# Skeletus/SC-GameEngine

Hardware: AMD Instinct MI355X
Metric: entities/sec world-tick (xform+broadphase+cull), 1M-entity world (higher is better)
Workload: dtype f32

## Files before the change

### sc_gameengine_amd/csrc/sc_tick_kernels.hip

```cpp
#include "sc_tick_internal.h"
#include <hip/hip_ext.h>
#include "../../include/sc_tick.h"


namespace sctick {

#ifndef SC_XFORM_OCC
#define SC_XFORM_OCC
#endif
#ifndef SC_ROW_STORE_POLICY
#define SC_ROW_STORE_POLICY 2
#endif
#ifndef SC_WAVE_CHAINS
#define SC_WAVE_CHAINS 1
#endif
#ifndef SC_PAIR_OCC
#define SC_PAIR_OCC __attribute__((amdgpu_waves_per_eu(5, 5)))
#endif
#ifndef SC_PX_STORE_POLICY_TILE
#define SC_PX_STORE_POLICY_TILE 2
#endif
#ifndef SC_PX_STORE_POLICY_TAIL
#define SC_PX_STORE_POLICY_TAIL 0
#endif
#ifndef SC_DIAG_CLASSED_TAIL
#define SC_DIAG_CLASSED_TAIL 0
#endif

struct Aff { float r0[4], r1[4], r2[4]; };

__device__ __forceinline__ bool dirtyBit(const uint32_t* __restrict__ bits, uint32_t i)
{
  return (bits[i >> 5] >> (i & 31u)) & 1u;
}

__device__ __forceinline__ float ldF(const DeviceState& d, uint32_t stream, uint32_t i)
{
  return *reinterpret_cast<const float*>(d.fslab + (stream * d.capBytes + i * 4u));
}
__device__ __forceinline__ uint32_t ldU(const DeviceState& d, uint32_t stream, uint32_t i)
{
  return *reinterpret_cast<const uint32_t*>(d.fslab + (stream * d.capBytes + i * 4u));
}
__device__ __forceinline__ float4 ldRow(const DeviceState& d, uint32_t row, uint32_t i)
{
  return *reinterpret_cast<const float4*>(d.rslab + (row * d.capBytes16 + i * 16u));
}
typedef float V4f __attribute__((ext_vector_type(4)));
__device__ __forceinline__ void stRow(const DeviceState& d, uint32_t row, uint32_t i, const float4& v)
{
  *reinterpret_cast<float4*>(d.rslab + (row * d.capBytes16 + i * 16u)) = v;
}
__device__ __forceinline__ void stRowPolicy(const DeviceState& d, uint32_t row, uint32_t i, const float4& v)
{
#if SC_ROW_STORE_POLICY == 0
  stRow(d, row, i, v);
#else
  const V4f x = { v.x, v.y, v.z, v.w };
  const uint32_t off = row * d.capBytes16 + i * 16u;
#if SC_ROW_STORE_POLICY == 1
  __builtin_nontemporal_store(x, reinterpret_cast<V4f*>(d.rslab + off));
#elif SC_ROW_STORE_POLICY == 2
  asm volatile("global_store_dwordx4 %0, %1, %2 sc1" : : "v"(off), "v"(x), "s"(d.rslab) : "memory");
#elif SC_ROW_STORE_POLICY == 3
  asm volatile("global_store_dwordx4 %0, %1, %2 sc0 sc1" : : "v"(off), "v"(x), "s"(d.rslab) : "memory");
#else
#error "SC_ROW_STORE_POLICY: 0 plain, 1 nt, 2 sc1, 3 sc0 sc1"
#endif
#endif
}
template <int kPolicy>
__device__ __forceinline__ void stPxPolicy(const DeviceState& d, uint32_t i, float v)
{
  static_assert(kPolicy == 0 || kPolicy == 2, "px store policy: 0 plain, 2 sc1");
  if constexpr (kPolicy == 0) d.px[i] = v;
  else asm volatile("global_store_dword %0, %1, %2 sc1" : : "v"(i * 4u), "v"(v), "s"(d.px) : "memory");
}

__device__ __forceinline__ Aff loadLocal(const DeviceState& d, uint32_t j, uint32_t lkj)
{
  const uint32_t triv = lkj >> 29;
  float sx = 0.0f, cx = 1.0f, sy = 0.0f, cy = 1.0f, sz = 0.0f, cz = 1.0f;
  if (!(triv & 1u)) { sx = ldF(d, kRSX, j); cx = ldF(d, kRCX, j); }
  if (!(triv & 2u)) { sy = ldF(d, kRSY, j); cy = ldF(d, kRCY, j); }
  if (!(triv & 4u)) { sz = ldF(d, kRSZ, j); cz = ldF(d, kRCZ, j); }
  const float kx = ldF(d, kSX, j), ky = ldF(d, kSY, j), kz = ldF(d, kSZ, j);
  const float a00 = cz * cy, a10 = sz * cy, a20 = -sy;
  const float a01 = -sz,     a11 = cz;
  const float a02 = cz * sy, a12 = sz * sy, a22 = cy;
  const float nsx = -sx;
  const float r01 = a01 * cx + a02 * sx, r11 = a11 * cx + a12 * sx, r21 = a22 * sx;
  const float r02 = a01 * nsx + a02 * cx, r12 = a11 * nsx + a12 * cx, r22 = a22 * cx;
  Aff L;
  L.r0[0] = a00 * kx; L.r0[1] = r01 * ky; L.r0[2] = r02 * kz; L.r0[3] = ldF(d, kPX, j);
  L.r1[0] = a10 * kx; L.r1[1] = r11 * ky; L.r1[2] = r12 * kz; L.r1[3] = ldF(d, kPY, j);
  L.r2[0] = a20 * kx; L.r2[1] = r21 * ky; L.r2[2] = r22 * kz; L.r2[3] = ldF(d, kPZ, j);
  return L;
}
struct LocalRaw { float sx, cx, sy, cy, sz, cz, kx, ky, kz, px, py, pz; };
__device__ __forceinline__ LocalRaw requestLocal(const DeviceState& d, uint32_t j, uint32_t lkj)
{
  const uint32_t triv = lkj >> 29;
  LocalRaw r;
  r.sx = 0.0f; r.cx = 1.0f; r.sy = 0.0f; r.cy = 1.0f; r.sz = 0.0f; r.cz = 1.0f;
  if (!(triv & 1u)) { r.sx = ldF(d, kRSX, j); r.cx = ldF(d, kRCX, j); }
  if (!(triv & 2u)) { r.sy = ldF(d, kRSY, j); r.cy = ldF(d, kRCY, j); }
  if (!(triv & 4u)) { r.sz = ldF(d, kRSZ, j); r.cz = ldF(d, kRCZ, j); }
  r.kx = ldF(d, kSX, j); r.ky = ldF(d, kSY, j); r.kz = ldF(d, kSZ, j);
  r.px = ldF(d, kPX, j); r.py = ldF(d, kPY, j); r.pz = ldF(d, kPZ, j);
  return r;
}
__device__ __forceinline__ Aff buildLocal(const LocalRaw& q)
{
  const float a00 = q.cz * q.cy, a10 = q.sz * q.cy, a20 = -q.sy;
  const float a01 = -q.sz,       a11 = q.cz;
  const float a02 = q.cz * q.sy, a12 = q.sz * q.sy, a22 = q.cy;
  const float nsx = -q.sx;
  const float r01 = a01 * q.cx + a02 * q.sx, r11 = a11 * q.cx + a12 * q.sx, r21 = a22 * q.sx;
  const float r02 = a01 * nsx + a02 * q.cx, r12 = a11 * nsx + a12 * q.cx, r22 = a22 * q.cx;
  Aff L;
  L.r0[0] = a00 * q.kx; L.r0[1] = r01 * q.ky; L.r0[2] = r02 * q.kz; L.r0[3] = q.px;
  L.r1[0] = a10 * q.kx; L.r1[1] = r11 * q.ky; L.r1[2] = r12 * q.kz; L.r1[3] = q.py;
  L.r2[0] = a20 * q.kx; L.r2[1] = r21 * q.ky; L.r2[2] = r22 * q.kz; L.r2[3] = q.pz;
  return L;
}

__device__ __forceinline__ void mulRow(const float p[4], const Aff& L, float out[4])
{
  out[0] = (p[0] * L.r0[0] + p[1] * L.r1[0]) + p[2] * L.r2[0];
  out[1] = (p[0] * L.r0[1] + p[1] * L.r1[1]) + p[2] * L.r2[1];
  out[2] = (p[0] * L.r0[2] + p[1] * L.r1[2]) + p[2] * L.r2[2];
  out[3] = ((p[0] * L.r0[3] + p[1] * L.r1[3]) + p[2] * L.r2[3]) + p[3];
}
__device__ __forceinline__ Aff mulAff(const Aff& P, const Aff& L)
{
  Aff W;
  mulRow(P.r0, L, W.r0); mulRow(P.r1, L, W.r1); mulRow(P.r2, L, W.r2);
  return W;
}

__device__ __forceinline__ Aff loadRows(const DeviceState& d, uint32_t j)
{
  const float4 a = ldRow(d, 0, j), b = ldRow(d, 1, j), c = ldRow(d, 2, j);
  Aff M;
  M.r0[0] = a.x; M.r0[1] = a.y; M.r0[2] = a.z; M.r0[3] = a.w;
  M.r1[0] = b.x; M.r1[1] = b.y; M.r1[2] = b.z; M.r1[3] = b.w;
  M.r2[0] = c.x; M.r2[1] = c.y; M.r2[2] = c.z; M.r2[3] = c.w;
  return M;
}
__device__ __forceinline__ void storeRows(const DeviceState& d, uint32_t j, const Aff& M)
{
  stRow(d, 0, j, make_float4(M.r0[0], M.r0[1], M.r0[2], M.r0[3]));
  stRow(d, 1, j, make_float4(M.r1[0], M.r1[1], M.r1[2], M.r1[3]));
  stRow(d, 2, j, make_float4(M.r2[0], M.r2[1], M.r2[2], M.r2[3]));
}
__device__ __forceinline__ void storeRowsPolicy(const DeviceState& d, uint32_t j, const Aff& M)
{
  stRowPolicy(d, 0, j, make_float4(M.r0[0], M.r0[1], M.r0[2], M.r0[3]));
  stRowPolicy(d, 1, j, make_float4(M.r1[0], M.r1[1], M.r1[2], M.r1[3]));
  stRowPolicy(d, 2, j, make_float4(M.r2[0], M.r2[1], M.r2[2], M.r2[3]));
}

__device__ __forceinline__ float fromLane(int src4, float v) { return __int_as_float(__builtin_amdgcn_ds_bpermute(src4, __float_as_int(v))); }
__device__ __forceinline__ Aff affFromLane(int src4, const Aff& M)
{
  Aff P;
#pragma unroll
  for (int c = 0; c < 4; ++c) { P.r0[c] = fromLane(src4, M.r0[c]); P.r1[c] = fromLane(src4, M.r1[c]); P.r2[c] = fromLane(src4, M.r2[c]); }
  return P;
}

struct BoundsCE { float cx, cy, cz, ex, ey, ez; };
__device__ __forceinline__ BoundsCE loadBounds(const DeviceState& d, uint32_t j)
{
  const float x0 = ldF(d, kBMINX, j), y0 = ldF(d, kBMINY, j), z0 = ldF(d, kBMINZ, j);
  const float x1 = ldF(d, kBMAXX, j), y1 = ldF(d, kBMAXY, j), z1 = ldF(d, kBMAXZ, j);
  BoundsCE b;
  b.cx = (x0 + x1) * 0.5f; b.cy = (y0 + y1) * 0.5f; b.cz = (z0 + z1) * 0.5f;
  b.ex = (x1 - x0) * 0.5f; b.ey = (y1 - y0) * 0.5f; b.ez = (z1 - z0) * 0.5f;
  return b;
}
typedef const __attribute__((address_space(4))) float* ConstF;
typedef const __attribute__((address_space(4))) uint32_t* ConstU;
__device__ __forceinline__ BoundsCE paletteBounds(ConstF e)
{
  const float x0 = e[0], y0 = e[1], z0 = e[2], x1 = e[3], y1 = e[4], z1 = e[5];
  BoundsCE b;
  b.cx = (x0 + x1) * 0.5f; b.cy = (y0 + y1) * 0.5f; b.cz = (z0 + z1) * 0.5f;
  b.ex = (x1 - x0) * 0.5f; b.ey = (y1 - y0) * 0.5f; b.ez = (z1 - z0) * 0.5f;
  return b;
}

__device__ __forceinline__ bool sphereVisibleAt(const Aff& M, const BoundsCE& b, ConstF fr)
{
  const float c0 = M.r0[0] * b.cx + M.r0[1] * b.cy + M.r0[2] * b.cz + M.r0[3];
  const float c1 = M.r1[0] * b.cx + M.r1[1] * b.cy + M.r1[2] * b.cz + M.r1[3];
  const float c2 = M.r2[0] * b.cx + M.r2[1] * b.cy + M.r2[2] * b.cz + M.r2[3];
  const float nx = M.r0[0] * M.r0[0] + M.r1[0] * M.r1[0] + M.r2[0] * M.r2[0];
  const float ny = M.r0[1] * M.r0[1] + M.r1[1] * M.r1[1] + M.r2[1] * M.r2[1];
  const float nz = M.r0[2] * M.r0[2] + M.r1[2] * M.r1[2] + M.r2[2] * M.r2[2];
  const float nyz = (ny < nz) ? nz : ny;
  const float maxScale = sqrtf((nx < nyz) ? nyz : nx);
  const float radius = sqrtf(b.ex * b.ex + b.ey * b.ey + b.ez * b.ez) * maxScale;
  bool out = false;
#pragma unroll
  for (int k = 0; k < 6; ++k) {
    const float dist = fr[4 * k] * c0 + fr[4 * k + 1] * c1 + fr[4 * k + 2] * c2 + fr[4 * k + 3];
    out = out || (dist < -radius);
  }
  return !out;
}

__device__ __forceinline__ void worldAabb(const Aff& M, const BoundsCE& b, float mn[3], float mx[3])
{
  const float c0 = M.r0[0] * b.cx + M.r0[1] * b.cy + M.r0[2] * b.cz + M.r0[3];
  const float c1 = M.r1[0] * b.cx + M.r1[1] * b.cy + M.r1[2] * b.cz + M.r1[3];
  const float c2 = M.r2[0] * b.cx + M.r2[1] * b.cy + M.r2[2] * b.cz + M.r2[3];
  const float h0 = fabsf(M.r0[0]) * b.ex + fabsf(M.r0[1]) * b.ey + fabsf(M.r0[2]) * b.ez;
  const float h1 = fabsf(M.r1[0]) * b.ex + fabsf(M.r1[1]) * b.ey + fabsf(M.r1[2]) * b.ez;
  const float h2 = fabsf(M.r2[0]) * b.ex + fabsf(M.r2[1]) * b.ey + fabsf(M.r2[2]) * b.ez;
  mn[0] = c0 - h0; mn[1] = c1 - h1; mn[2] = c2 - h2;
  mx[0] = c0 + h0; mx[1] = c1 + h1; mx[2] = c2 + h2;
}

__device__ __forceinline__ void colliderAabb(const Aff& M, const float4& s, uint32_t type, float mn[3], float mx[3])
{
  float pad = 0.0f;
  if (type != kColliderBox) {
    const float nx = M.r0[0] * M.r0[0] + M.r1[0] * M.r1[0] + M.r2[0] * M.r2[0];
    const float ny = M.r0[1] * M.r0[1] + M.r1[1] * M.r1[1] + M.r2[1] * M.r2[1];
    const float nz = M.r0[2] * M.r0[2] + M.r1[2] * M.r1[2] + M.r2[2] * M.r2[2];
    const float nyz = (type == kColliderSphere && nz < ny) ? ny : nz;
    pad = s.w * sqrtf((nx < nyz) ? nyz : nx);
  }
  const float h0 = fabsf(M.r0[0]) * s.x + fabsf(M.r0[1]) * s.y + fabsf(M.r0[2]) * s.z + pad;
  const float h1 = fabsf(M.r1[0]) * s.x + fabsf(M.r1[1]) * s.y + fabsf(M.r1[2]) * s.z + pad;
  const float h2 = fabsf(M.r2[0]) * s.x + fabsf(M.r2[1]) * s.y + fabsf(M.r2[2]) * s.z + pad;
  mn[0] = M.r0[3] - h0; mn[1] = M.r1[3] - h1; mn[2] = M.r2[3] - h2;
  mx[0] = M.r0[3] + h0; mx[1] = M.r1[3] + h1; mx[2] = M.r2[3] + h2;
}
__device__ __forceinline__ bool hasProxy(uint32_t type, bool hasBounds) { return type == kColliderBounds ? hasBounds : type != kColliderNone; }
__device__ __forceinline__ bool proxyAabb(const DeviceState& d, uint32_t i, uint32_t lk, const Aff& M, float mn[3], float mx[3])
{
  const uint32_t type = d.colType ? d.colType[i] : kColliderBounds;
  if (!hasProxy(type, (lk & kHasBounds) != 0u)) return false;
  if (type == kColliderBounds) { const BoundsCE b = loadBounds(d, i); worldAabb(M, b, mn, mx); }
  else colliderAabb(M, d.colShape[i], type, mn, mx);
  return true;
}

struct BinPlan { bool collide, big; float x0, z0; uint32_t nx, nz; };

__device__ __forceinline__ BinPlan planBins(const TickParams& p, const float mn[3], const float mx[3])
{
  BinPlan b; b.collide = false; b.big = false; b.x0 = b.z0 = 0.0f; b.nx = b.nz = 0;
  if (!(mn[0] == mn[0] && mn[1] == mn[1] && mn[2] == mn[2] && mx[0] == mx[0] && mx[1] == mx[1] && mx[2] == mx[2])) return b;
  b.collide = true;
  const float x0 = floorf(mn[0] * p.invSector) - p.binOx, x1 = floorf(mx[0] * p.invSector) - p.binOx;
  const float z0 = floorf(mn[2] * p.invSector) - p.binOz, z1 = floorf(mx[2] * p.invSector) - p.binOz;
  const float nx = x1 - x0 + 1.0f, nz = z1 - z0 + 1.0f;
  const bool ok = x0 >= 0.0f && z0 >= 0.0f && x1 < (float)p.binSX && z1 < (float)p.binSZ &&
                  nx >= 1.0f && nx <= 2.0f && nz >= 1.0f && nz <= 2.0f;
  if (!ok) { b.big = true; return b; }
  b.x0 = x0; b.z0 = z0; b.nx = (uint32_t)nx; b.nz = (uint32_t)nz;
  return b;
}

__device__ __forceinline__ void appendBig(const DeviceState& d, const TickParams& p, const float4& rmin, const float4& rmax)
{
  const uint32_t slot = atomicAdd(&d.counters[kCtrPar + 8u * p.parity + kCtrBig], 1u);
  if (slot >= p.bigCap) return;
  d.bigList[2u * (size_t)slot] = rmin;
  d.bigList[2u * (size_t)slot + 1u] = rmax;
}

__device__ __forceinline__ void queueCrowded(const DeviceState& d, const TickParams& p, uint32_t sector)
{
  const uint32_t at = atomicAdd(&d.counters[kCtrPar + 8u * p.parity + kCtrCrowdTail], 1u);
  const uint32_t sectors = p.binSX * p.binSZ;
  if (at < sectors) d.crowdQueue[p.parity * sectors + at] = sector;
}

__device__ __forceinline__ void binInsertLane(const DeviceState& d, const TickParams& p, uint32_t sector, const float4& rmin, const float4& rm)
{
  const uint32_t slot = atomicAdd(&d.binCount[sector], 1u);
  atomicOr(&d.binLayers[sector], __float_as_uint(rmin.w));
  if (slot < kBinCap) {
    float4* r = d.bins + 2u * ((size_t)sector * kBinCap + slot);
    r[0] = rmin; r[1] = rm;
  } else {
    if (slot == kBinCap) queueCrowded(d, p, sector);
    const uint32_t ctr = kCtrPar + 8u * p.parity;
    const uint32_t at = atomicAdd(&d.counters[ctr + kCtrSpill], 1u);
    if (at < p.ovfCap) {
      d.spill[2u * (size_t)at] = rmin; d.spill[2u * (size_t)at + 1u] = rm; d.spillSector[at] = sector;
      atomicMin(&d.ovfLo[sector], at); atomicMax(&d.ovfHi[sector], at + 1u);
    } else atomicAdd(&d.counters[ctr + kCtrBorderLost], 1u);
  }
}

__device__ __forceinline__ void nullRecord(float4& lo, float4& hi, uint32_t id = 0x00FFFFFFu)
{
  lo = make_float4(INFINITY, INFINITY, INFINITY, __uint_as_float(0u));
  hi = make_float4(-INFINITY, -INFINITY, -INFINITY, __uint_as_float(id));
}

__host__ __device__ __forceinline__ uint32_t layersThatCanMeet(uint32_t H, uint32_t V)
{
  V |= H;
  const bool meet = ((V & 0xFFFFu) & (H >> 16)) != 0u && ((H & 0xFFFFu) & (V >> 16)) != 0u;
  return meet ? 0xFFFFFFFFu : 0u;
}
__device__ __forceinline__ bool binWrittenEveryTick(uint32_t homeLayers, uint32_t sector, uint32_t binSX, uint32_t binSZ)
{
  const uint32_t gx = sector % binSX, gz = sector / binSX;
  return ((homeLayers & 0xFFFFu) & (homeLayers >> 16)) != 0u || gx == 0u || gz == 0u || gx + 1u == binSX || gz + 1u == binSZ;
}

__device__ __forceinline__ void spillLane(const DeviceState& d, const TickParams& p, uint32_t sector, uint32_t slot, const float4& rmin, const float4& rm)
{
  if (slot == kBinCap) queueCrowded(d, p, sector);
  const uint32_t ctr = kCtrPar + 8u * p.parity;
  const uint32_t at = atomicAdd(&d.counters[ctr + kCtrSpill], 1u);
  if (at < p.ovfCap) {
    d.spill[2u * (size_t)at] = rmin; d.spill[2u * (size_t)at + 1u] = rm; d.spillSector[at] = sector;
    atomicMin(&d.ovfLo[sector], at); atomicMax(&d.ovfHi[sector], at + 1u);
  } else atomicAdd(&d.counters[ctr + kCtrBorderLost], 1u);
}

template <uint32_t kHome, bool kColl>
__device__ __forceinline__ void binEntityWave(const DeviceState& d, const TickParams& p, uint32_t i, bool collider,
                                              const Aff& M, const BoundsCE& b, bool storeM, bool lazyOn, uint32_t tile0, uint32_t tile1, uint32_t ctype)
{
  float mn[3] = {0, 0, 0}, mx[3] = {0, 0, 0};
  BinPlan plan; plan.collide = false; plan.big = false; plan.x0 = plan.z0 = 0.0f; plan.nx = plan.nz = 0;
  float4 rmin = make_float4(0, 0, 0, 0), rmax = make_float4(0, 0, 0, 0);
  constexpr uint32_t mode = kHome;
  uint32_t hA = kNoHome, hB = 0xFFFFFFFFu;
  if (mode == kHomeUse && i < p.n) { hA = d.homeA[i]; hB = d.homeB[i]; }
  if (collider) {
    if (kColl && ctype != kColliderBounds) colliderAabb(M, d.colShape[i], ctype, mn, mx);
    else worldAabb(M, b, mn, mx);
    plan = planBins(p, mn, mx);
    rmin = make_float4(mn[0], mn[1], mn[2], __uint_as_float((tile0 & kTileLayersShared) ? tile1 : ldU(d, kLAYERS, i)));
    rmax = make_float4(mx[0], mx[1], mx[2], __uint_as_float(i | p.rankBits));
  }
  const bool want = plan.collide && !plan.big;
  const uint32_t sector = (uint32_t)plan.z0 * p.binSX + (uint32_t)plan.x0;
  const uint32_t lane = threadIdx.x & 63u;
  const bool atHome = want && hA == sector;
  const bool r0 = atHome && (hB & 0xFFu) != kNoSlot;
  const bool a0 = want && !r0;
  uint32_t slot = hB & kSlotMask;
  const bool stay = p.cleanStay != 0u && !storeM;
  const bool skip0 = r0 && ((hB & kSlotAlways) ? stay : lazyOn);
  float4 rm = rmax;
  rm.w = __uint_as_float(i | p.rankBits | kPrimary);
  const uint32_t myLay = __float_as_uint(rmin.w);

  const unsigned long long act = ballot64(a0);
  uint32_t myHead = lane, runEnd = lane + 1u;
  if (act) {
    const uint32_t key = a0 ? sector : 0xFFFFFFFFu;
    const uint32_t prev = __shfl_up(key, 1, 64);
    const bool head = a0 && (lane == 0 || prev != key);
    const unsigned long long heads = ballot64(head);
    const unsigned long long upto = (lane == 63u) ? ~0ull : ((2ull << lane) - 1ull);
    myHead = (63u - (uint32_t)__clzll(heads & upto)) & 63u;
    const unsigned long long above = (myHead == 63u) ? 0ull : ~((2ull << myHead) - 1ull);
    const unsigned long long ends = (heads | ~act) & above;
    runEnd = ends ? (uint32_t)__ffsll((long long)ends) - 1u : 64u;
    uint32_t lay = a0 ? myLay : 0u;
    const uint32_t headLay = (uint32_t)__shfl((int)lay, (int)myHead, 64);
    if (ballot64(a0 && headLay != lay)) {
#pragma unroll
      for (uint32_t o = 1; o < 64u; o <<= 1) {
        const uint32_t other = (uint32_t)__shfl_down((int)lay, o, 64);
        if (a0 && lane + o < runEnd) lay |= other;
      }
    }
    uint32_t base = 0;
    if (head) { base = atomicAdd(&d.binCount[sector], runEnd - lane); atomicOr(&d.binLayers[sector], lay); }
    if (storeM) storeRows(d, i, M);
    base = __shfl(base, myHead, 64);
    if (a0) slot = base + (lane - myHead);
  } else if (storeM) storeRows(d, i, M);
  if (want && slot < kBinCap && !skip0) {
    float4* r = d.bins + 2u * ((size_t)sector * kBinCap + slot);
    r[0] = rmin; r[1] = rm;
  }
  uint32_t learned = (want && slot < kBinCap) ? slot : kNoSlot;
  const bool c1 = want && plan.nx > 1u, c2 = want && plan.nz > 1u, c3 = c1 && c2;
  if (mode == kHomeUse) {
    const uint32_t sec1 = sector + 1u, sec2 = sector + p.binSX, sec3 = sec2 + 1u;
    const uint32_t b1 = (hB >> 8) & 0xFFu, b2 = (hB >> 16) & 0xFFu, b3 = hB >> 24;
    uint32_t q1 = b1 & kSlotMask, q2 = b2 & kSlotMask, q3 = b3 & kSlotMask;
    const bool h1 = atHome && b1 != kNoSlot, h2 = atHome && b2 != kNoSlot, h3 = atHome && b3 != kNoSlot;
    const bool a1 = c1 && !h1, a2 = c2 && !h2, a3 = c3 && !h3;
    const bool w1 = c1 && !(h1 && ((b1 & kSlotAlways) ? stay : lazyOn)), w2 = c2 && !(h2 && ((b2 & kSlotAlways) ? stay : lazyOn)),
               w3 = c3 && !(h3 && ((b3 & kSlotAlways) ? stay : lazyOn));
    if (a1) q1 = atomicAdd(&d.binCount[sec1], 1u);
    if (a2) q2 = atomicAdd(&d.binCount[sec2], 1u);
    if (a3) q3 = atomicAdd(&d.binCount[sec3], 1u);
    if (w1 && q1 < kBinCap) { float4* r = d.bins + 2u * ((size_t)sec1 * kBinCap + q1); r[0] = rmin; r[1] = rmax; }
    if (w2 && q2 < kBinCap) { float4* r = d.bins + 2u * ((size_t)sec2 * kBinCap + q2); r[0] = rmin; r[1] = rmax; }
    if (w3 && q3 < kBinCap) { float4* r = d.bins + 2u * ((size_t)sec3 * kBinCap + q3); r[0] = rmin; r[1] = rmax; }
    if (a1) atomicOr(&d.binLayers[sec1], myLay);
    if (a2) atomicOr(&d.binLayers[sec2], myLay);
    if (a3) atomicOr(&d.binLayers[sec3], myLay);
    if (ballot64((a1 && q1 >= kBinCap) || (a2 && q2 >= kBinCap) || (a3 && q3 >= kBinCap))) {
      if (a1 && q1 >= kBinCap) spillLane(d, p, sec1, q1, rmin, rmax);
      if (a2 && q2 >= kBinCap) spillLane(d, p, sec2, q2, rmin, rmax);
      if (a3 && q3 >= kBinCap) spillLane(d, p, sec3, q3, rmin, rmax);
    }
    if (hA != kNoHome && !(atHome && c1 && c2)) {
      float4 lo, hi; nullRecord(lo, hi, i | p.rankBits);
#pragma unroll
      for (uint32_t k = 0; k < 4u; ++k) {
        const bool ck = k == 0u ? want : (k == 1u ? c1 : (k == 2u ? c2 : c3));
        const uint32_t gk = (hB >> (8u * k)) & 0xFFu;
        if (gk != kNoSlot && !(atHome && ck) && !(lazyOn && !(gk & kSlotAlways))) {
          float4* r = d.bins + 2u * ((size_t)(hA + (k & 1u) + (k >> 1) * p.binSX) * kBinCap + (gk & kSlotMask)); r[0] = lo; r[1] = hi;
        }
      }
    }
  } else {
    const uint32_t sec1 = sector + 1u, sec2 = sector + p.binSX, sec3 = sec2 + 1u;
    uint32_t q1 = 0, q2 = 0, q3 = 0;
    if (c1) q1 = atomicAdd(&d.binCount[sec1], 1u);
    if (c2) q2 = atomicAdd(&d.binCount[sec2], 1u);
    if (c3) q3 = atomicAdd(&d.binCount[sec3], 1u);
    if (c1 && q1 < kBinCap) { float4* r = d.bins + 2u * ((size_t)sec1 * kBinCap + q1); r[0] = rmin; r[1] = rmax; }
    if (c2 && q2 < kBinCap) { float4* r = d.bins + 2u * ((size_t)sec2 * kBinCap + q2); r[0] = rmin; r[1] = rmax; }
    if (c3 && q3 < kBinCap) { float4* r = d.bins + 2u * ((size_t)sec3 * kBinCap + q3); r[0] = rmin; r[1] = rmax; }
    if (c1) atomicOr(&d.binLayers[sec1], myLay);
    if (c2) atomicOr(&d.binLayers[sec2], myLay);
    if (c3) atomicOr(&d.binLayers[sec3], myLay);
    learned |= ((c1 && q1 < kBinCap ? q1 : kNoSlot) << 8) | ((c2 && q2 < kBinCap ? q2 : kNoSlot) << 16) | ((c3 && q3 < kBinCap ? q3 : kNoSlot) << 24);
    if (ballot64((c1 && q1 >= kBinCap) || (c2 && q2 >= kBinCap) || (c3 && q3 >= kBinCap))) {
      if (c1 && q1 >= kBinCap) spillLane(d, p, sec1, q1, rmin, rmax);
      if (c2 && q2 >= kBinCap) spillLane(d, p, sec2, q2, rmin, rmax);
      if (c3 && q3 >= kBinCap) spillLane(d, p, sec3, q3, rmin, rmax);
    }
    if (mode == kHomeLearn && i < p.n) { d.homeA[i] = want ? sector : kNoHome; d.homeB[i] = learned; }
  }
  const bool over = a0 && slot >= kBinCap;
  const unsigned long long mo = ballot64(over);
  if (mo) {
    const uint32_t ctr = kCtrPar + 8u * p.parity;
    const uint32_t first = (uint32_t)__ffsll((long long)mo) - 1u;
    uint32_t at = 0;
    if (lane == first) at = atomicAdd(&d.counters[ctr + kCtrSpill], (uint32_t)__popcll(mo));
    at = __shfl(at, (int)first, 64) + (uint32_t)__popcll(mo & ((1ull << lane) - 1ull));
    if (over && slot == kBinCap) queueCrowded(d, p, sector);
    if (over && at < p.ovfCap) {
      d.spill[2u * (size_t)at] = rmin; d.spill[2u * (size_t)at + 1u] = rm; d.spillSector[at] = sector;
      if (slot == kBinCap || lane == myHead) atomicMin(&d.ovfLo[sector], at);
      if (lane + 1u == runEnd) atomicMax(&d.ovfHi[sector], at + 1u);
    } else if (over) atomicAdd(&d.counters[ctr + kCtrBorderLost], 1u);
  }
  if (plan.collide && plan.big) appendBig(d, p, rmin, rmax);
}

__device__ __forceinline__ void binBoxSingle(const DeviceState& d, const TickParams& p, uint32_t i, const float mn[3], const float mx[3])
{
  const BinPlan plan = planBins(p, mn, mx);
  const float4 rmin = make_float4(mn[0], mn[1], mn[2], __uint_as_float(ldU(d, kLAYERS, i)));
  float4 rmax = make_float4(mx[0], mx[1], mx[2], __uint_as_float(i | p.rankBits));
  if (!plan.collide) return;
  if (plan.big) { appendBig(d, p, rmin, rmax); return; }
  const uint32_t sx = (uint32_t)plan.x0, sz = (uint32_t)plan.z0;
  for (uint32_t k = 0; k < 4; ++k) {
    const uint32_t dx = k & 1u, dz = k >> 1;
    if (!(dx < plan.nx && dz < plan.nz)) continue;
    float4 rm = rmax; if (k == 0) rm.w = __uint_as_float(i | p.rankBits | kPrimary);
    binInsertLane(d, p, (sz + dz) * p.binSX + (sx + dx), rmin, rm);
  }
}

__device__ __forceinline__ void binEntitySingle(const DeviceState& d, const TickParams& p, uint32_t i, const Aff& M, const BoundsCE& b)
{
  float mn[3], mx[3];
  worldAabb(M, b, mn, mx);
  binBoxSingle(d, p, i, mn, mx);
}

template <bool kCull, bool kAabb, uint32_t kChain, uint32_t kHome, bool kColl, bool kTail = false>
__device__ __forceinline__ void xformCullBody(const DeviceState& d, const TickParams& p);

__device__ __forceinline__ void spanTail(const DeviceState& d, const TickParams& p, uint32_t begin, uint32_t end, uint32_t tid)
{
  if (begin >= end) return;
  const bool produce = (p.flags & SC_TICK_PRODUCE_NEXT) != 0;
  const uint32_t wBegin = begin >> 5, wEnd = (end + 31u) >> 5;
  const uint32_t w = wBegin + tid;
  const uint32_t wAt = w < wEnd ? w : wEnd - 1u;
  const uint32_t dw = d.dirty[wAt], uw = d.unreach[wAt];
  uint32_t rw = 0u;
  if (produce) rw = d.rootMask[wAt];
  constexpr uint32_t kBatch = 3;
  uint32_t rm[kBatch]; float x[kBatch];
  if (produce) {
#pragma unroll
    for (uint32_t u = 0; u < kBatch; ++u) {
      const uint32_t i = begin + u * kTile + tid;
      const uint32_t at = i < end ? i : end - 1u;
      rm[u] = d.rootMask[at >> 5];
      x[u] = d.px[at];
    }
  }
  __syncthreads();
  if (produce) {
#pragma unroll
    for (uint32_t u = 0; u < kBatch; ++u) {
      const uint32_t i = begin + u * kTile + tid;
      if (i < end && ((rm[u] >> (i & 31u)) & 1u)) stPxPolicy<SC_PX_STORE_POLICY_TAIL>(d, i, x[u] + p.producerParam);
    }
    for (uint32_t base = begin + kBatch * kTile; base < end; base += kBatch * kTile) {
#pragma unroll
      for (uint32_t u = 0; u < kBatch; ++u) {
        const uint32_t i = base + u * kTile + tid;
        const uint32_t at = i < end ? i : end - 1u;
        rm[u] = d.rootMask[at >> 5];
        x[u] = d.px[at];
      }
#pragma unroll
      for (uint32_t u = 0; u < kBatch; ++u) {
        const uint32_t i = base + u * kTile + tid;
        if (i < end && ((rm[u] >> (i & 31u)) & 1u)) stPxPolicy<SC_PX_STORE_POLICY_TAIL>(d, i, x[u] + p.producerParam);
      }
    }
  }
  if (w < wEnd) d.dirty[w] = (dw & uw) | rw;
  for (uint32_t v = w + kTile; v < wEnd; v += kTile) d.dirty[v] = (d.dirty[v] & d.unreach[v]) | (produce ? d.rootMask[v] : 0u);
}

template <uint32_t kChain>
struct TileWalk {
  uint32_t lk;
  uint32_t a[kChain + 1];
  uint32_t rotFlags, cur;
  int top;
  uint32_t pendLink, pendDirty;
};
template <uint32_t kChain>
__device__ __forceinline__ void walkRequest(const DeviceState& d, TileWalk<kChain>& w, uint32_t i, uint32_t last)
{
  w.a[0] = i <= last ? i : last;
  w.pendLink = ldU(d, kLINK, w.a[0]);
  w.pendDirty = d.dirty[w.a[0] >> 5];
}
template <uint32_t kChain>
__device__ __forceinline__ void walkResolve(TileWalk<kChain>& w, uint32_t lev, uint32_t i, uint32_t last, bool doXform)
{
  asm volatile("" : : "v"(w.pendLink), "v"(w.pendDirty));
  if (lev == 0u) {
    w.lk = i <= last ? w.pendLink : ((kUnreachable << kDepthShift) | kNoParent);
    w.rotFlags = w.lk >> 29; w.cur = w.lk;
    const bool walk = doXform && linkDepth(w.lk) <= kChain;
    w.top = (walk && ((w.pendDirty >> (w.a[0] & 31u)) & 1u)) ? 0 : -1;
  } else {
    const uint32_t depth = linkDepth(w.lk);
    const bool on = doXform && depth <= kChain && lev <= depth;
    w.cur = on ? w.pendLink : w.cur;
    w.rotFlags |= on ? (w.pendLink >> 29) << (3u * lev) : 0u;
    w.top = (on && ((w.pendDirty >> (w.a[lev] & 31u)) & 1u)) ? (int)lev : w.top;
  }
}
template <uint32_t kChain>
__device__ __forceinline__ void walkIssue(const DeviceState& d, TileWalk<kChain>& w, uint32_t lev, bool doXform)
{
  const uint32_t depth = linkDepth(w.lk);
  const bool on = doXform && depth <= kChain && lev <= depth;
  w.a[lev] = on ? (w.cur & kParentMask) : w.a[0];
  w.pendLink = ldU(d, kLINK, w.a[lev]);
  w.pendDirty = d.dirty[w.a[lev] >> 5];
}

struct ClassPend { uint32_t tw0; uint2 ent, dm; };
__device__ __forceinline__ void classRequest(const DeviceState& d, ClassPend& np, uint32_t i, uint32_t last)
{
  const uint32_t a0 = i <= last ? i : last;
  const uint32_t t = __builtin_amdgcn_readfirstlane(a0 >> 6);
  np.tw0 = ((ConstU)d.boundsPalette)[kPaletteCap * 8u + 2u * t];
  np.dm = *reinterpret_cast<const uint2*>(d.dirty + 2u * (a0 >> 6));
}
__device__ __forceinline__ void classIssue(const DeviceState& d, ClassPend& np, uint32_t lane)
{
  const uint32_t pat = (np.tw0 >> kTopoShift) & kTopoMask;
  const uint32_t at = pat ? (pat <= kTopoCap ? pat - 1u : kTopoCap - 1u) : 0u;
  np.ent = topoTable(d.boundsPalette)[at * 64u + lane];
}
template <uint32_t kChain>
__device__ __forceinline__ void classResolve(const ClassPend& np, TileWalk<kChain>& w, uint32_t i, uint32_t last, uint32_t lane)
{
  asm volatile("" : : "v"(np.ent.x), "v"(np.dm.x), "v"(np.dm.y));
  const uint32_t pat = (np.tw0 >> kTopoShift) & kTopoMask;
  const uint32_t x = (i <= last && pat != 0u) ? np.ent.x : (kTopoInactive & 0xFF000000u);
  w.a[0] = i <= last ? i : last;
  w.lk = x; w.rotFlags = x >> 29; w.cur = x;
  const uint32_t depth = linkDepth(x);
  const bool walk = depth <= kChain;
  const unsigned long long dm = ((unsigned long long)np.dm.y << 32) | np.dm.x;
  int top = (walk && ((dm >> lane) & 1ull)) ? 0 : -1;
#pragma unroll
  for (uint32_t lev = 1; lev <= kChain; ++lev) {
    const uint32_t anc = (x >> (6u * (lev - 1u))) & 63u;
    top = (walk && lev <= depth && ((dm >> anc) & 1ull)) ? (int)lev : top;
  }
  w.top = top;
  if (kChain >= 1) w.a[kChain >= 1 ? 1 : 0] = (w.a[0] & ~63u) + (x & 63u);
}

template <bool kCull, uint32_t kChain, bool kTail, uint32_t kBatch = kChain + 1, bool kClassed = false>
__device__ __forceinline__ void xformCullPipelined(const DeviceState& d, const TickParams& p, const uint32_t bid = blockIdx.x)
{
  static_assert(kBatch >= 1 && kBatch <= kChain + 1, "levels requested together");
  static_assert(!kClassed || (SC_WAVE_CHAINS && kChain >= 1), "the classed form is the cooperative form");
  const uint32_t lane = threadIdx.x & 63u;
  const uint32_t wave = threadIdx.x >> 6;
  const uint32_t begin = bid * p.span;
  const uint32_t end = (begin + p.span < p.n) ? begin + p.span : p.n;
  const bool doXform = kClassed || (p.flags & SC_TICK_XFORM) != 0;
  const bool wantCand = (p.flags & SC_TICK_CULLED_LIST) != 0;
  const bool hasDeep = !kClassed && (p.flags & kFlagHasDeep) != 0;
  constexpr bool kEndInTile = kClassed && kTail;
  const bool produce = kEndInTile && !SC_DIAG_CLASSED_TAIL && (p.flags & SC_TICK_PRODUCE_NEXT) != 0;
  uint32_t tailWave = 0;
  if (kTail && !kCull && !kEndInTile) tailWave = __builtin_amdgcn_readfirstlane(wave);

  uint32_t visCount = 0, candCount = 0;
  TileWalk<kChain> w, nw;
  ClassPend np; uint32_t tw0 = 0u;

  auto tile = [&](uint32_t base, auto hasNext) {
    constexpr bool kNext = decltype(hasNext)::value;
    const uint32_t i = base + threadIdx.x;
    const uint32_t last = end - 1u;
    const bool active = i < p.n;
    const uint32_t lk = w.lk;
    const uint32_t depth = linkDepth(lk);
    const int top = w.top;
    const bool recompute = top >= 0;
    const bool fromRoot = (uint32_t)top == depth;

    uint32_t rows = i;
#pragma unroll
    for (uint32_t k = 0; k < kChain; ++k) if ((uint32_t)top == k) rows = w.a[k + 1];
    Aff M;
    auto walkAhead = [&]() {
      if constexpr (kClassed) { if (kNext) classRequest(d, np, i + kTile, last); }
      else if (kNext) { walkRequest(d, nw, i + kTile, last); walkResolve(nw, 0u, i + kTile, last, doXform); if (kChain >= 1) walkIssue(d, nw, 1u, doXform); }
    };
#if SC_WAVE_CHAINS
    bool coop = kClassed;
    if (!kClassed && kChain >= 1) coop = ballot64(top >= 1 && (w.a[kChain >= 1 ? 1 : 0] >> 6) != (i >> 6)) == 0ull;
    if (coop) {
      LocalRaw own;
      const bool nudge = produce && depth == 0u;
      if (recompute ? (top == 0 && !fromRoot) : (kCull && active)) M = loadRows(d, rows);
      if (recompute) own = requestLocal(d, w.a[0], w.rotFlags << 29);
      else if (kEndInTile && nudge) own.px = ldF(d, kPX, i);
      walkAhead();
      if (recompute) {
        const Aff L = buildLocal(own);
        if (top == 0 && !fromRoot) M = mulAff(M, L);
        else M = L;
      }
      if constexpr (kEndInTile && !SC_DIAG_CLASSED_TAIL) {
        if (nudge) stPxPolicy<SC_PX_STORE_POLICY_TILE>(d, i, own.px + p.producerParam);
        const unsigned long long nd = ballot64(nudge);
        if ((lane & 31u) == 0u && active) d.dirty[i >> 5] = (uint32_t)(nd >> lane);
      }
      const int src4 = (int)((top >= 1 ? (w.a[kChain >= 1 ? 1 : 0] & 63u) : lane) << 2);
#pragma unroll
      for (int pass = 1; pass <= (int)kChain; ++pass) {
        if (ballot64(top == pass) != 0ull) {
          const Aff P = affFromLane(src4, M);
          if (top == pass) M = mulAff(P, M);
        }
      }
    } else
#endif
    {
      if (recompute ? !fromRoot : (kCull && active)) M = loadRows(d, rows);
      LocalRaw raw[kChain + 1];
#pragma unroll
      for (int lev = (int)kChain; lev > (int)kChain - (int)kBatch; --lev)
        if (lev <= top) raw[lev] = requestLocal(d, w.a[lev], (w.rotFlags >> (3 * lev)) << 29);
      walkAhead();

      if (recompute) {
#pragma unroll
        for (int lev = (int)kChain; lev >= 0; --lev) {
          if (lev <= top) {
            if (lev <= (int)kChain - (int)kBatch) raw[lev] = requestLocal(d, w.a[lev], (w.rotFlags >> (3 * lev)) << 29);
            const Aff L = buildLocal(raw[lev]);
            if (lev == top && fromRoot) M = L;
            else M = mulAff(M, L);
          }
        }
      }
    }
    if constexpr (kClassed) { if (kNext) classIssue(d, np, lane); }
    else if (kNext && kChain >= 2) { walkResolve(nw, 1u, i + kTile, last, doXform); walkIssue(d, nw, 2u, doXform); }
    if (recompute) storeRowsPolicy(d, i, M);

    if (hasDeep) {
      const unsigned long long rm = ballot64(recompute);
      if (lane == 0 && (base + wave * 64u) < p.n) d.recomp[(base >> 6) + wave] = rm;
    }
    if (!kClassed && kNext && kChain >= 3) { walkResolve(nw, 2u, i + kTile, last, doXform); walkIssue(d, nw, 3u, doXform); }

    if (kCull) {
      const bool cand = active && (lk & kHasMesh);
      const bool hb = active && (lk & kHasBounds);
      const uint32_t t = __builtin_amdgcn_readfirstlane((base >> 6) + wave);
      ConstU tw = (ConstU)d.boundsPalette + (kPaletteCap * 8u + 2u * t);
      const uint32_t cls = (kClassed ? tw0 : tw[0]) & kClassMask;
      BoundsCE b = {0, 0, 0, 0, 0, 0};
      if (cls < kPaletteCap) b = paletteBounds((ConstF)d.boundsPalette + 8u * cls);
      else if (hb) b = loadBounds(d, i);

      bool visible = cand;
      if (cand && hb && !p.freeze && p.frustumValid) {
        const float* fr = d.frustum;
        asm volatile("" : "+s"(fr));
        visible = sphereVisibleAt(M, b, (ConstF)fr);
      }
      if (!kClassed && doXform && depth > kChain && depth != kUnreachable) visible = false;
      const unsigned long long vm = ballot64(visible);
      const unsigned long long cm = ballot64(cand);
      if (lane == 0 && (base + wave * 64u) < p.n) {
        d.vis[(base >> 6) + wave] = vm;
        if (wantCand) d.cand[(base >> 6) + wave] = cm;
      }
      visCount += (uint32_t)__popcll(vm);
      candCount += (uint32_t)__popcll(cm);
    }
    if constexpr (kClassed) { if (kNext) { classResolve(np, w, i + kTile, last, lane); tw0 = np.tw0; } }
    else if (kNext) { walkResolve(nw, kChain, i + kTile, last, doXform); w = nw; }
  };

  if (begin < end) {
    const uint32_t i0 = begin + threadIdx.x, last = end - 1u;
    if constexpr (kClassed) { classRequest(d, np, i0, last); classIssue(d, np, lane); classResolve(np, w, i0, last, lane); tw0 = np.tw0; }
    else {
      walkRequest(d, w, i0, last);
#pragma unroll
      for (uint32_t k = 1; k <= kChain; ++k) { walkResolve(w, k - 1u, i0, last, doXform); walkIssue(d, w, k, doXform); }
      walkResolve(w, kChain, i0, last, doXform);
    }
    uint32_t base = begin;
    for (; base + kTile < end; base += kTile) tile(base, std::true_type{});
    tile(base, std::false_type{});
  }

  if (kCull) {
    __shared__ uint32_t sVis[kTile / 64], sCand[kTile / 64];
    if (lane == 0) { sVis[wave] = visCount; sCand[wave] = candCount; }
    __syncthreads();
    if (threadIdx.x == 0) {
      d.blockVis[bid] = sVis[0] + sVis[1] + sVis[2] + sVis[3];
      d.blockCand[bid] = sCand[0] + sCand[1] + sCand[2] + sCand[3];
    }
  }
  if constexpr (kTail && !kEndInTile) spanTail(d, p, begin, end, kCull ? (wave << 6) + lane : (tailWave << 6) + __builtin_amdgcn_mbcnt_hi(~0u, __builtin_amdgcn_mbcnt_lo(~0u, 0u)));
}

#if SC_WAVE_CHAINS
constexpr uint32_t pipelinedBatch(bool, uint32_t) { return 1u; }
#else
constexpr uint32_t pipelinedBatch(bool cull, uint32_t chain) { return (cull && chain == 3u) ? 3u : chain + 1u; }
#endif

template <bool kCull, bool kAabb, uint32_t kChain, uint32_t kHome>
__global__ __launch_bounds__(kTile) SC_XFORM_OCC void k_xform_cull(const DeviceState d, const TickParams p)
{
  if constexpr (kAabb) xformCullBody<kCull, kAabb, kChain, kHome, false>(d, p);
  else xformCullPipelined<kCull, kChain, false, pipelinedBatch(kCull, kChain)>(d, p);
}
template <bool kCull, uint32_t kChain, uint32_t kHome>
__global__ __launch_bounds__(kTile) SC_XFORM_OCC void k_xform_cull_colliders(const DeviceState d, const TickParams p) { xformCullBody<kCull, true, kChain, kHome, true>(d, p); }
template <bool kCull, bool kAabb, uint32_t kChain, uint32_t kHome>
__global__ __launch_bounds__(kTile) SC_XFORM_OCC void k_xform_cull_tail(const DeviceState d, const TickParams p)
{
  if constexpr (kAabb) xformCullBody<kCull, kAabb, kChain, kHome, false, true>(d, p);
  else xformCullPipelined<kCull, kChain, true, pipelinedBatch(kCull, kChain)>(d, p);
}
template <bool kCull, uint32_t kChain>
__global__ __launch_bounds__(kTile) SC_XFORM_OCC void k_xform_cull_classed(const DeviceState d, const TickParams p) { xformCullPipelined<kCull, kChain, false, 1u, true>(d, p); }
template <bool kCull, uint32_t kChain>
__global__ __launch_bounds__(kTile) SC_XFORM_OCC void k_xform_cull_classed_tail(const DeviceState d, const TickParams p) { xformCullPipelined<kCull, kChain, true, 1u, true>(d, p); }
template <bool kCull, uint32_t kChain, uint32_t kHome>
__global__ __launch_bounds__(kTile) SC_XFORM_OCC void k_xform_cull_colliders_tail(const DeviceState d, const TickParams p) { xformCullBody<kCull, true, kChain, kHome, true, true>(d, p); }

template <bool kCull, bool kAabb, uint32_t kChain, uint32_t kHome, bool kColl, bool kTail>
__device__ __forceinline__ void xformCullBody(const DeviceState& d, const TickParams& p)
{
  const uint32_t lane = threadIdx.x & 63u;
  const uint32_t wave = threadIdx.x >> 6;
  const uint32_t begin = blockIdx.x * p.span;
  const uint32_t end = (begin + p.span < p.n) ? begin + p.span : p.n;
  const bool doXform = (p.flags & SC_TICK_XFORM) != 0;
  const bool wantCand = (p.flags & SC_TICK_CULLED_LIST) != 0;
  const bool hasDeep = (p.flags & kFlagHasDeep) != 0;
  uint32_t tailWave = 0;
  if (kTail && !kCull) tailWave = __builtin_amdgcn_readfirstlane(wave);

  uint32_t visCount = 0, candCount = 0;
  bool lazyOn = false;
  if (kAabb) {
    lazyOn = kHome == kHomeUse && (p.lazy == 2u || (p.lazy == 1u && d.lazyCtl[0] == 0u));
  }

  for (uint32_t base = begin; base < end; base += kTile) {
    const uint32_t i = base + threadIdx.x;
    const bool active = i < p.n;
    const uint32_t lk = active ? ldU(d, kLINK, i) : ((kUnreachable << kDepthShift) | kNoParent);
    const uint32_t ownDirtyWord = (doXform && active) ? d.dirty[i >> 5] : 0u;
    const uint32_t depth = linkDepth(lk);
    const bool chain = depth <= kChain;
    uint32_t a[kChain + 1];
    uint32_t rotFlags = lk >> 29;
    a[0] = i;
    int top = -1;
    if (doXform && chain) {
      if ((ownDirtyWord >> (i & 31u)) & 1u) top = 0;
      uint32_t cur = lk;
#pragma unroll
      for (uint32_t k = 1; k <= kChain; ++k) {
        a[k] = i;
        if (k <= depth) {
          a[k] = cur & kParentMask;
          cur = ldU(d, kLINK, a[k]);
          rotFlags |= (cur >> 29) << (3u * k);
          if (dirtyBit(d.dirty, a[k])) top = (int)k;
        }
      }
    } else {
#pragma unroll
      for (uint32_t k = 1; k <= kChain; ++k) a[k] = i;
    }
    const bool recompute = top >= 0;

    Aff M;
    if (recompute) {
      const bool fromRoot = (uint32_t)top == depth;
      uint32_t seed = i;
#pragma unroll
      for (uint32_t k = 0; k < kChain; ++k) if ((uint32_t)top == k) seed = a[k + 1];
      if (!fromRoot) M = loadRows(d, seed);
#pragma unroll
      for (int lev = (int)kChain; lev >= 0; --lev) {
        if (lev <= top) {
          const Aff L = loadLocal(d, a[lev], (rotFlags >> (3 * lev)) << 29);
          if (lev == top && fromRoot) M = L;
          else M = mulAff(M, L);
        }
      }
      if (!kAabb) storeRows(d, i, M);
    } else if ((kCull || kAabb) && active) {
      M = loadRows(d, i);
    }

    if (hasDeep) {
      const unsigned long long rm = ballot64(recompute);
      if (lane == 0 && (base + wave * 64u) < p.n) d.recomp[(base >> 6) + wave] = rm;
    }

    if (kCull || kAabb) {
      const bool cand = active && (lk & kHasMesh);
      const bool hb = active && (lk & kHasBounds);
      uint32_t ctype = kColliderNone;
      if (kColl && active) ctype = d.colType[i];
      const uint32_t t = __builtin_amdgcn_readfirstlane((base >> 6) + wave);
      ConstU tw = (ConstU)d.boundsPalette + (kPaletteCap * 8u + 2u * t);
      const uint32_t tile0 = tw[0], tile1 = kAabb ? tw[1] : 0u;
      const uint32_t cls = tile0 & kClassMask;
      BoundsCE b = {0, 0, 0, 0, 0, 0};
      if (cls < kPaletteCap) b = paletteBounds((ConstF)d.boundsPalette + 8u * cls);
      else if (hb) b = loadBounds(d, i);

      if (kCull) {
        bool visible = cand;
        if (cand && hb && !p.freeze && p.frustumValid) {
          const float* fr = d.frustum;
          asm volatile("" : "+s"(fr));
          visible = sphereVisibleAt(M, b, (ConstF)fr);
        }
        if (doXform && depth > kChain && depth != kUnreachable) visible = false;
        const unsigned long long vm = ballot64(visible);
        const unsigned long long cm = ballot64(cand);
        if (lane == 0 && (base + wave * 64u) < p.n) {
          d.vis[(base >> 6) + wave] = vm;
          if (wantCand) d.cand[(base >> 6) + wave] = cm;
        }
        visCount += (uint32_t)__popcll(vm);
        candCount += (uint32_t)__popcll(cm);
      }
      if (kAabb) {
        const bool collider = (kColl ? hasProxy(ctype, hb) : hb) && !(doXform && depth > kChain && depth != kUnreachable);
        binEntityWave<kHome, kColl>(d, p, i, collider, M, b, recompute, lazyOn, tile0, tile1, ctype);
      }
    }
  }

  if (kAabb && blockIdx.x == 0 && threadIdx.x == 0) d.lazyCtl[1u + p.parity] = lazyOn ? 0u : 1u;
  if (kCull) {
    __shared__ uint32_t sVis[kTile / 64], sCand[kTile / 64];
    if (lane == 0) { sVis[wave] = visCount; sCand[wave] = candCount; }
    __syncthreads();
    if (threadIdx.x == 0) {
      d.blockVis[blockIdx.x] = sVis[0] + sVis[1] + sVis[2] + sVis[3];
      d.blockCand[blockIdx.x] = sCand[0] + sCand[1] + sCand[2] + sCand[3];
    }
  }
  if (kTail) spanTail(d, p, begin, end, kCull ? (wave << 6) + lane : (tailWave << 6) + __builtin_amdgcn_mbcnt_hi(~0u, __builtin_amdgcn_mbcnt_lo(~0u, 0u)));
}

template <bool kColl>
__device__ __forceinline__ void deepLevelBody(const DeviceState& d, const TickParams& p, const uint32_t* __restrict__ list, uint32_t count)
{
  const uint32_t t = blockIdx.x * kTile + threadIdx.x;
  if (t >= count) return;
  const uint32_t i = list[t];
  const uint32_t lk = ldU(d, kLINK, i);
  const uint32_t par = lk & kParentMask;
  bool nodeDirty = false;
  Aff M;
  if (p.flags & SC_TICK_XFORM) {
    nodeDirty = dirtyBit(d.dirty, i) || ((d.recomp[par >> 6] >> (par & 63u)) & 1ull);
    if (nodeDirty) {
      const Aff P = loadRows(d, par);
      const Aff L = loadLocal(d, i, lk);
      M = mulAff(P, L);
      storeRows(d, i, M);
      atomicOr((unsigned long long*)&d.recomp[i >> 6], 1ull << (i & 63u));
    }
  }
  if (!nodeDirty) M = loadRows(d, i);
  const bool hb = (lk & kHasBounds) != 0;
  BoundsCE b = {0, 0, 0, 0, 0, 0};
  if (hb) b = loadBounds(d, i);
  if (p.flags & SC_TICK_CULL) {
    bool visible = (lk & kHasMesh) != 0;
    if (visible && hb && !p.freeze && p.frustumValid) visible = sphereVisibleAt(M, b, (ConstF)d.frustum);
    if (visible) {
      atomicOr((unsigned long long*)&d.vis[i >> 6], 1ull << (i & 63u));
      atomicAdd(&d.blockVis[i / p.span], 1u);
    }
  }
  if (p.flags & SC_TICK_BROADPHASE) {
    if (kColl) { float mn[3], mx[3]; if (proxyAabb(d, i, lk, M, mn, mx)) binBoxSingle(d, p, i, mn, mx); }
    else if (hb) binEntitySingle(d, p, i, M, b);
  }
}
__global__ __launch_bounds__(kTile) void k_deep_level(const DeviceState d, const TickParams p, const uint32_t* __restrict__ list, uint32_t count) { deepLevelBody<false>(d, p, list, count); }
__global__ __launch_bounds__(kTile) void k_deep_level_colliders(const DeviceState d, const TickParams p, const uint32_t* __restrict__ list, uint32_t count) { deepLevelBody<true>(d, p, list, count); }

__device__ __forceinline__ bool nudgePosition(const DeviceState& d, uint32_t i, uint32_t n, float dx)
{
  const bool in = i < n;
  const uint32_t lk = in ? d.link[i] : ((kUnreachable << kDepthShift) | 1u);
  const float x = in ? d.px[i] : 0.0f;
  const bool root = in && (lk & kParentMask) == kNoParent && linkDepth(lk) != kUnreachable;
  if (root) d.px[i] = x + dx;
  return root;
}
__device__ __forceinline__ void markDirtyWave(const DeviceState& d, uint32_t i, uint32_t n, bool moved)
{
  const uint32_t lane = threadIdx.x & 63u;
  const unsigned long long m = ballot64(moved);
  const uint32_t mine = lane < 32u ? (uint32_t)m : (uint32_t)(m >> 32);
  if (i < n && (lane & 31u) == 0u && mine) d.dirty[i >> 5] |= mine;
}
struct LaneStep { bool ok; uint32_t lane; float s; float pos[3]; float dir[3]; };
__device__ __forceinline__ LaneStep advanceAlongLane(const LaneGraphDev& g, uint32_t lane, float s, float distance)
{
  LaneStep r; r.ok = false; r.lane = lane; r.s = s;
  r.pos[0] = r.pos[1] = r.pos[2] = 0.0f; r.dir[0] = r.dir[1] = r.dir[2] = 0.0f;
  if (lane == kInvalidLane || lane >= g.segments) return r;
  float remaining = distance; uint32_t current = lane; float currentS = s;
  for (uint32_t guard = 0; guard < 8u; ++guard) {
    const float4 A = g.segA[current], B = g.segB[current]; const uint4 C = g.segC[current];
    if (!C.y) return r;
    const float len = A.w;
    if (len <= 1e-5f) return r;
    const float available = len - currentS;
    if (remaining <= available) {
      currentS += remaining;
      r.pos[0] = A.x + B.x * currentS; r.pos[1] = A.y + B.y * currentS; r.pos[2] = A.z + B.z * currentS;
      r.dir[0] = B.x; r.dir[1] = B.y; r.dir[2] = B.z;
      r.lane = current; r.s = currentS; r.ok = true;
      return r;
    }
    remaining -= available; currentS = 0.0f;
    uint32_t best = kInvalidLane; float bestDot = -1.0f;
    const uint32_t c0 = g.nodeConnOff[C.x], c1 = g.nodeConnOff[C.x + 1u];
    for (uint32_t k = c0; k < c1; ++k) {
      const uint32_t segId = g.nodeConn[k];
      if (segId >= g.segments) continue;
      if (!g.segC[segId].y) continue;
      const float4 D = g.segB[segId];
      const float dot = B.x * D.x + B.y * D.y + B.z * D.z;
      if (dot > bestDot) { bestDot = dot; best = segId; }
    }
    if (best == kInvalidLane) {
      const float4 E = g.nodePos[C.x];
      r.pos[0] = E.x; r.pos[1] = E.y; r.pos[2] = E.z; r.dir[0] = B.x; r.dir[1] = B.y; r.dir[2] = B.z;
      r.lane = current; r.s = len; r.ok = true;
      return r;
    }
    current = best;
  }
  return r;
}

__device__ __forceinline__ uint32_t queryNearestLaneWave(const LaneGraphDev& g, float x, float y, float z, float& sOut)
{
  const uint32_t lane = threadIdx.x & 63u;
  float bestD = INFINITY, bestS = 0.0f; uint32_t best = kInvalidLane;
  for (uint32_t i = lane; i < g.segments; i += 64u) {
    const uint4 C = g.segC[i];
    const float4 A = g.segA[i], B = g.segB[i];
    if (!C.y || A.w <= 1e-5f) continue;
    const float tx = x - A.x, ty = y - A.y, tz = z - A.z;
    const float proj = tx * B.x + ty * B.y + tz * B.z;
    const float mn = (proj < A.w) ? proj : A.w;
    const float sv = (0.0f < mn) ? mn : 0.0f;
    const float cx = A.x + B.x * sv, cy = A.y + B.y * sv, cz = A.z + B.z * sv;
    const float dx = x - cx, dy = y - cy, dz = z - cz;
    const float distSq = dx * dx + dy * dy + dz * dz;
    if (best == kInvalidLane || distSq < bestD) { bestD = distSq; best = i; bestS = sv; }
  }
  unsigned long long key = ((unsigned long long)__float_as_uint(bestD) << 32) | best;
  unsigned long long low = key;
#pragma unroll
  for (int o = 32; o > 0; o >>= 1) { const unsigned long long other = __shfl_xor(low, o, 64); low = other < low ? other : low; }
  const unsigned long long winners = ballot64(best != kInvalidLane && key == low);
  sOut = 0.0f;
  if (!winners) return kInvalidLane;
  const int win = __ffsll((long long)winners) - 1;
  sOut = __shfl(bestS, win, 64);
  return (uint32_t)__shfl((int)best, win, 64);
}

__device__ __forceinline__ bool trafficAgentStep(const DeviceState& d, uint32_t i, uint32_t lane, float s0, float dt, float smooth, float mult)
{
  if (d.aMode[i] != kTierOnRails) return false;
  const LaneGraphDev& g = d.lanes;
  if (lane == kInvalidLane || lane >= g.segments) return false;
  if (!g.segC[lane].y) return false;
  const LaneStep look = advanceAlongLane(g, lane, s0, d.aLook[i]);
  if (!look.ok) return false;
  const float tx = look.pos[0] - d.px[i], tz = look.pos[2] - d.pz[i];
  if (sqrtf(tx * tx + 0.0f * 0.0f + tz * tz) < 1e-4f) return false;
  float desiredSpeed = g.segB[lane].w * mult;
  desiredSpeed = (0.0f < desiredSpeed) ? desiredSpeed : 0.0f;
  const float obstacleBrake = d.aBrake ? d.aBrake[i] : 0.0f;
  const float desired = desiredSpeed * (1.0f - obstacleBrake);
  const float cur = d.aSpeed[i];
  const float speed = cur + (desired - cur) * smooth;
  d.aSpeed[i] = speed;
  const LaneStep st = advanceAlongLane(g, lane, s0, speed * dt);
  if (!st.ok) return false;
  d.aLane[i] = st.lane; d.aS[i] = st.s;
  d.px[i] = st.pos[0]; d.pz[i] = st.pos[2];
  const uint4 C = g.segC[st.lane];
  d.rsx[i] = 0.0f; d.rcx[i] = 1.0f; d.rsy[i] = __uint_as_float(C.z); d.rcy[i] = __uint_as_float(C.w); d.rsz[i] = 0.0f; d.rcz[i] = 1.0f;
  return true;
}

__device__ __forceinline__ bool moverPosition(const DeviceState& d, uint32_t i, uint32_t n, float dt, float smooth, float mult)
{
  const bool in = i < n;
  const uint32_t kind = in ? d.moverKind[i] : 0u;
  float vx = 0, vz = 0, lox = 0, loz = 0, hix = 0, hiz = 0, x = 0, z = 0;
  if (in) { vx = d.mvx[i]; vz = d.mvz[i]; lox = d.mlox[i]; loz = d.mloz[i]; hix = d.mhix[i]; hiz = d.mhiz[i]; x = d.px[i]; z = d.pz[i]; }
  uint32_t aLane = kInvalidLane; float aS = 0.0f;
  if (d.aLane) {
    const bool agent = kind == kMoverTraffic;
    if (agent) { aLane = d.aLane[i]; aS = d.aS[i]; }
    unsigned long long lost = ballot64(agent && aLane == kInvalidLane);
    while (lost) {
      const int src = __ffsll((long long)lost) - 1;
      lost &= lost - 1ull;
      const uint32_t who = (uint32_t)__shfl((int)i, src, 64);
      float qs;
      const uint32_t q = queryNearestLaneWave(d.lanes, __shfl(x, src, 64), d.py[who], __shfl(z, src, 64), qs);
      if ((int)(threadIdx.x & 63u) == src && q != kInvalidLane) { aLane = q; aS = qs; d.aLane[i] = q; d.aS[i] = qs; }
    }
  }
  if (kind == kMoverTraffic) return trafficAgentStep(d, i, aLane, aS, dt, smooth, mult);
  if (kind) {
    x = x + vx * dt; z = z + vz * dt;
    if (kind == 1u) {
      if (x >= hix) x = lox + (x - hix); else if (x < lox) x = hix - (lox - x);
      if (z >= hiz) z = loz + (z - hiz); else if (z < loz) z = hiz - (loz - z);
    } else {
      if (x > hix) { x = hix - (x - hix); vx = -vx; } else if (x < lox) { x = lox + (lox - x); vx = -vx; }
      if (z > hiz) { z = hiz - (z - hiz); vz = -vz; } else if (z < loz) { z = loz + (loz - z); vz = -vz; }
      d.mvx[i] = vx; d.mvz[i] = vz;
    }
    d.px[i] = x; d.pz[i] = z;
  }
  return kind != 0u;
}
__device__ __forceinline__ bool producePosition(const DeviceState& d, const TickParams& p, uint32_t i)
{
  return p.producerKind == 1u ? nudgePosition(d, i, p.n, p.producerParam) : moverPosition(d, i, p.n, p.producerParam, p.trafficSmooth, p.trafficMult);
}

constexpr uint32_t kCompactScratch = 4u * (kTile / 64u);
__device__ __forceinline__ uint4 blockSum4(uint4 v, uint32_t* scratch)
{
#pragma unroll
  for (int o = 32; o > 0; o >>= 1) {
    v.x += __shfl_down(v.x, o, 64); v.y += __shfl_down(v.y, o, 64); v.z += __shfl_down(v.z, o, 64); v.w += __shfl_down(v.w, o, 64);
  }
  const uint32_t lane = threadIdx.x & 63u, wave = threadIdx.x >> 6;
  __syncthreads();
  if (lane == 0) reinterpret_cast<uint4*>(scratch)[wave] = v;
  __syncthreads();
  uint4 r = make_uint4(0, 0, 0, 0);
#pragma unroll
  for (uint32_t k = 0; k < kTile / 64u; ++k) {
    const uint4 q = reinterpret_cast<const uint4*>(scratch)[k];
    r.x += q.x; r.y += q.y; r.z += q.z; r.w += q.w;
  }
  return r;
}

#ifndef SC_DIAG_EOT
#define SC_DIAG_EOT 0
#endif
constexpr uint32_t kCompactWordsMax = kTile;
constexpr uint32_t kCompactLdsWords = kCompactWordsMax * 6u;

__device__ __forceinline__ void emitVisible(const DeviceState& d, const TickParams& p, uint32_t off, uint32_t j)
{
  float4* items = reinterpret_cast<float4*>(p.emitTarget);
  if (p.emitMode == 2u) {
    if (off < p.emitMaxVisible) p.emitTarget[kFrameHeaderWords + off] = j;
    items = reinterpret_cast<float4*>(frameItems(p.emitTarget, p.emitMaxVisible));
  }
  if (p.emitBudget == 0u || off < p.emitBudget) {
    const float4 a = ldRow(d, 0, j), b = ldRow(d, 1, j), c = ldRow(d, 2, j);
    writeDrawItem(d, items + 5u * (size_t)off, j, a, b, c);
  }
}

template <bool kEmit>
__device__ __forceinline__ void compactBody(const DeviceState& d, const TickParams& p, uint32_t bid, uint32_t nblocks, uint32_t group,
                                            uint32_t* scratch, uint32_t* moved, uint32_t* words)
{
  const uint32_t lane = threadIdx.x & 63u;
  const uint32_t wave = threadIdx.x >> 6;
  const uint32_t width = p.span * group;
  const uint32_t begin = bid * width;
  const uint32_t end = (begin + width < p.n) ? begin + width : p.n;
  const bool doCull = (p.flags & SC_TICK_CULL) != 0;
  const bool doCulled = (p.flags & SC_TICK_CULLED_LIST) != 0;

  const uint32_t wBegin = begin >> 5, wEnd = (end + 31u) >> 5;
  const uint32_t dirtyWord = wBegin + threadIdx.x;
  const bool tailOwns = (p.flags & kFlagTailOwnsDirty) != 0;
// ... 1924 lines not shown
```

Before: 65.01 billion.

## Compose parent transforms across lanes within a wave instead of reloading parent rows

When every dirty entity in a wave has its parent in the same 64-entity wave, each lane computes only its own local matrix. Parent world matrices are then pulled from the parent's lane through cross-lane shuffles, one pass per chain level. This avoids global loads of parent rows and the redundant recomputation of ancestor chains. The cost is extra ballots and shuffle passes, plus a compile-time predicate that restricts which kernel variants use the path.

```diff
diff --git a/sc_gameengine_amd/csrc/sc_tick_kernels.hip b/sc_gameengine_amd/csrc/sc_tick_kernels.hip
--- a/sc_gameengine_amd/csrc/sc_tick_kernels.hip
+++ b/sc_gameengine_amd/csrc/sc_tick_kernels.hip
@@ -13,6 +13,9 @@
 #endif
 #ifndef SC_WAVE_CHAINS
 #define SC_WAVE_CHAINS 1
+#endif
+#ifndef SC_BIN_WAVE_CHAINS
+#define SC_BIN_WAVE_CHAINS 1
 #endif
 #ifndef SC_PAIR_OCC
 #define SC_PAIR_OCC __attribute__((amdgpu_waves_per_eu(5, 5)))
@@ -487,6 +490,13 @@
 
 template <bool kCull, bool kAabb, uint32_t kChain, uint32_t kHome, bool kColl, bool kTail = false>
 __device__ __forceinline__ void xformCullBody(const DeviceState& d, const TickParams& p);
+constexpr bool binWaveChains(bool cull, uint32_t chain, uint32_t home, bool coll, bool tail)
+{
+  if (home != kHomeUse) return true;
+  if (chain == 1u) return !(cull ? !tail : (coll ? !tail : tail));
+  if (chain == 2u) return cull || coll;
+  return true;
+}
 
 __device__ __forceinline__ void spanTail(const DeviceState& d, const TickParams& p, uint32_t begin, uint32_t end, uint32_t tid)
 {
@@ -805,6 +815,7 @@
   const bool doXform = (p.flags & SC_TICK_XFORM) != 0;
   const bool wantCand = (p.flags & SC_TICK_CULLED_LIST) != 0;
   const bool hasDeep = (p.flags & kFlagHasDeep) != 0;
+  constexpr bool kCoop = SC_BIN_WAVE_CHAINS && kChain >= 1 && binWaveChains(kCull, kChain, kHome, kColl, kTail);
   uint32_t tailWave = 0;
   if (kTail && !kCull) tailWave = __builtin_amdgcn_readfirstlane(wave);
 
@@ -845,24 +856,45 @@
     const bool recompute = top >= 0;
 
     Aff M;
+    bool coop = false;
+    if constexpr (kCoop) {
+      const bool up = top >= 1;
+      if (ballot64(up) != 0ull) coop = ballot64(up && (a[kChain >= 1 ? 1 : 0] >> 6) != (i >> 6)) == 0ull;
+    }
+    const int mine = (coop && top > 0) ? 0 : top;
+    const int src4 = (int)((top >= 1 ? (a[kChain >= 1 ? 1 : 0] & 63u) : lane) << 2);
+    bool inPass[kChain + 1];
+#pragma unroll
+    for (int pass = 1; pass <= (int)kChain; ++pass) inPass[pass] = coop && top == pass;
     if (recompute) {
-      const bool fromRoot = (uint32_t)top == depth;
+      const bool fromRoot = mine != top || (uint32_t)top == depth;
       uint32_t seed = i;
 #pragma unroll
-      for (uint32_t k = 0; k < kChain; ++k) if ((uint32_t)top == k) seed = a[k + 1];
+      for (uint32_t k = 0; k < kChain; ++k) if ((uint32_t)mine == k) seed = a[k + 1];
       if (!fromRoot) M = loadRows(d, seed);
 #pragma unroll
       for (int lev = (int)kChain; lev >= 0; --lev) {
-        if (lev <= top) {
+        if (lev <= mine) {
           const Aff L = loadLocal(d, a[lev], (rotFlags >> (3 * lev)) << 29);
-          if (lev == top && fromRoot) M = L;
+          if (lev == mine && fromRoot) M = L;
           else M = mulAff(M, L);
         }
       }
-      if (!kAabb) storeRows(d, i, M);
     } else if ((kCull || kAabb) && active) {
       M = loadRows(d, i);
     }
+    if constexpr (kCoop) {
+      if (coop) {
+#pragma unroll
+        for (int pass = 1; pass <= (int)kChain; ++pass) {
+          if (pass == 1 || ballot64(inPass[pass]) != 0ull) {
+            const Aff P = affFromLane(src4, M);
+            if (inPass[pass]) M = mulAff(P, M);
+          }
+        }
+      }
+    }
+    if (!kAabb && recompute) storeRows(d, i, M);
 
     if (hasDeep) {
       const unsigned long long rm = ballot64(recompute);
```

After: 65.02 billion (median of 3 runs). About the same (+0.0%).
